# ExaScience/bpmf

Hardware: AMD Instinct MI355X
Metric: user+item column samples/sec per Gibbs iter; test RMSE vs reference (higher is better)
Workload: dtype f64

## Files before the change

### bpmf_amd/csrc/args.h

```cpp
#pragma once
#include <hip/hip_runtime.h>
#include <stdint.h>

#include "blob.h"

namespace bpmf {

__host__ __device__ constexpr int tri_off(int i) { return 2 * ((i >> 1) + 1) * ((i >> 1) + (i & 1)); }

template <int K>
struct Geo {
    static constexpr int NT = (K + 15) / 16;
    static constexpr int NTRI = NT * (NT + 1) / 2;
    static constexpr int PART = NTRI * 256 + NT * 16;
    static constexpr int WPS = K <= 32 ? 4 : 2;
    static constexpr int C = 64 / K;
    static constexpr int NP = K / 2;
    static constexpr int PLEN = tri_off(K);
    static constexpr int SLOT = PLEN + 2 * K;
    static constexpr int LDS_WORDS = C * SLOT + 2 * C;
};

template <int K>
struct Geo44 {
    static constexpr int NG = K / 4;
    static constexpr int NB = NG * (NG + 1) / 2;
    static constexpr int NL = K / 8;
    static constexpr int PART = (NB + NG) * 64;
    __host__ __device__ static constexpr int idx(int g, int x) { return 8 * (g >> 1) + 2 * x + (g & 1); }
};

struct SampleArgs {
    const int32_t *rowidx;
    const double *vals;
    const int32_t *wi_col;
    const int64_t *wi_p0;
    const int32_t *wi_len;
    const int32_t *wi_mc;
    const int32_t *wi_chunk;
    const int32_t *mc_slot0;
    const int32_t *mc_nchunks;
    unsigned *mc_count;
    double *partials;
    int nwork;
    const double *other_items;
    const double *zero_row;
    double *items;
    int64_t col_from;
    const double *LambdaF;
    const double *Lmu;
    const double *mu;
    const float *lf32;
    const double *prop_lambda;
    uint32_t diag_only;
    unsigned long long *fail;
    double mean_rating;
    double alpha;
    uint32_t iter_plus_1;
    int ktrue;
    const unsigned *gate_flag;
    unsigned gate_want;
    unsigned long long *tmo;
    unsigned long long wait_ticks;
    unsigned long long *stamps;
    uint32_t ablate;
};

struct FusedArgs {
    const unsigned *gate_host; unsigned gate_want; const double *src_host; double *dst; int n; unsigned *dflag; unsigned dval;
    int nstat; const double *st_items; int64_t st_c0, st_c1; double *st_partials; const unsigned long long *st_fail;
    double *st_out; unsigned *st_ticket; unsigned *st_flag; unsigned st_seq;
    unsigned long long *st_tmo;
// ... 51 lines not shown
```

### bpmf_amd/csrc/capi_side.hip

```cpp
#include "capi_internal.h"

namespace bpmf_capi {

int build_schedule(bpmf_hip_side *s, const int64_t *colptr)
{
    const int64_t nloc = s->to - s->from;
    const int K = s->ctx->K;
    const int mode_env = env_int("BPMF_HIP_MODE", -1);
    const bool f32 = s->ctx->dtype == BPMF_HIP_F32;
    const bool big = K == 128;
    if (big) s->mode = 5;
    else if (K == 64) s->mode = 4;
    else s->mode = (mode_env == 1 || mode_env == 3) ? mode_env : (nloc >= 20000 ? 3 : 1);
    int chunk = env_int("BPMF_HIP_CHUNK", 0);
    if (chunk <= 0) {
        const int64_t simds = (int64_t)s->ctx->num_cu * 4;
        int64_t c = s->mode == 4 ? (s->nnz * 9) / (simds * 16) : (s->mode == 5 ? (s->nnz * (f32 ? 3 : 6)) / (simds * 7) : s->nnz / simds);
        c = (c + 63) / 64 * 64;
        const int64_t lo = s->mode == 4 ? 256 : (s->mode == 5 ? 256 : 16 * K);
        chunk = (int)std::min<int64_t>(std::max<int64_t>(c, lo), 65536);
        if (s->mode == 3) chunk = std::max(chunk / 4, 4 * K);
    }
    chunk = (chunk + 15) / 16 * 16;
    s->chunk = chunk;

    struct Item { int32_t col; int64_t p0; int32_t len; int32_t mc; int32_t chunk; int64_t cost; };
    std::vector<Item> items;
    items.reserve((size_t)nloc + (size_t)(s->nnz / chunk) + 16);
    std::vector<int32_t> mc_slot0, mc_nch;
    const int64_t fin_cost = 32;
    int32_t slots = 0;
    for (int64_t c = 0; c < nloc; ++c) {
        const int64_t p0 = colptr[c], n = colptr[c + 1] - colptr[c];
        if (n < 0) return fail(BPMF_HIP_EINVAL, "colptr is not monotone");
        if (n <= chunk) {
// ... 60 lines not shown
        if (pfmax > 0) {
            size_t at[18] = {0};
            for (const Item &it : items)
                if (it.mc < 0 && it.len <= pfmax) at[it.len + 1]++;
            for (int n = 1; n <= pfmax + 1; ++n) at[n] += at[n - 1];
            lc.resize(at[pfmax + 1]); ll.resize(at[pfmax + 1]); lp.resize(at[pfmax + 1]);
            if (pfmax >= 3) s->pf_class[1] = (int)at[4];
            if (pfmax >= 6) s->pf_class[2] = (int)at[7];
            for (const Item &it : items)
                if (it.mc < 0 && it.len <= pfmax) { const size_t q = at[it.len]++; lc[q] = it.col; ll[q] = it.len; lp[q] = it.p0; }
        }
        s->pf_ratings = s->pf_ratings2 = 0;
        for (int32_t l : ll) { s->pf_ratings += l; s->pf_ratings2 += (int64_t)l * l; }
        if (pfmax < 3) s->pf_class[1] = (int)lc.size();
        if (pfmax < 6) s->pf_class[2] = (int)lc.size();
        s->pf_class[3] = (int)lc.size();
        for (const Item &it : items)
            if (!(it.mc < 0 && it.len <= nlr)) { hc.push_back(it.col); hl.push_back(it.len); hm.push_back(it.mc); hk.push_back(it.chunk); hp.push_back(it.p0); }
        if (nlr > 0 && (int64_t)lc.size() * 2 >= nloc && !lc.empty()) {
            s->lr_n = (int)lc.size(); s->hv_nwork = (int)hc.size();
            if (s->pf_class[3] > 0 && (rc = dev_upload<double>(&s->d_pf_q, nullptr, (size_t)s->nrows * K))) return rc;
            if ((rc = dev_upload(&s->d_lr_col, lc.data(), lc.size())) || (rc = dev_upload(&s->d_lr_len, ll.data(), ll.size())) ||
                (rc = dev_upload(&s->d_lr_p0, lp.data(), lp.size())) || (rc = dev_upload(&s->d_hv_col, hc.data(), hc.size())) ||
                (rc = dev_upload(&s->d_hv_len, hl.data(), hl.size())) || (rc = dev_upload(&s->d_hv_mc, hm.data(), hm.size())) ||
                (rc = dev_upload(&s->d_hv_chunk, hk.data(), hk.size())) || (rc = dev_upload(&s->d_hv_p0, hp.data(), hp.size())))
                return rc;
        }
    }
    if ((rc = dev_upload(&s->d_wi_col, wcol.data(), nw))) return rc;
    if ((rc = dev_upload(&s->d_wi_len, wlen.data(), nw))) return rc;
    if ((rc = dev_upload(&s->d_wi_mc, wmc.data(), nw))) return rc;
    if ((rc = dev_upload(&s->d_wi_chunk, wchunk.data(), nw))) return rc;
    if ((rc = dev_upload(&s->d_wi_p0, wp0.data(), nw))) return rc;
    if ((rc = dev_upload(&s->d_mc_slot0, mc_slot0.data(), mc_slot0.size()))) return rc;
    if ((rc = dev_upload(&s->d_mc_nch, mc_nch.data(), mc_nch.size()))) return rc;
    {
        std::vector<unsigned> zeros(std::max<size_t>(mc_slot0.size(), 8 * 32), 0u);
        if ((rc = dev_upload(&s->d_mc_count, zeros.data(), std::max<size_t>(mc_slot0.size(), 1)))) return rc;
    }
    if (big) {
        s->nstat_waves = (int)std::max<int64_t>(1, std::min<int64_t>((nloc + 63) / 64, 32));
        if ((rc = dev_upload<double>(&s->d_stat_partials, nullptr, (size_t)s->nstat_waves * blob::stat_partial_words(K)))) return rc;
        if ((rc = dev_upload<double>(&s->d_partials, nullptr, (size_t)slots * part_words_rt(K, f32)))) return rc;
        return 0;
    }
    const size_t pw = part_words_rt(K, false);
    if ((rc = dev_upload<double>(&s->d_partials, nullptr, (size_t)slots * pw))) return rc;
    s->nstat_waves = (int)std::max<int64_t>(1, std::min<int64_t>((nloc + 31) / 32, (int64_t)s->ctx->num_cu * (nloc > 100000 ? 8 : 2)));
    if (nloc < 20000) s->nstat_waves = (int)std::max<int64_t>(1, std::min<int64_t>(s->nstat_waves, std::max<int64_t>((nloc + 159) / 160, 24)));
    s->nstat_wg = (nloc > 100000) ? (int)std::min<int64_t>((nloc + 127) / 128, (int64_t)s->ctx->num_cu * 2) : 0;
    if ((rc = dev_upload<double>(&s->d_stat_partials, nullptr, (size_t)std::max(s->nstat_waves, 2 * s->nstat_wg) * pw))) return rc;
    return 0;
}

void free_schedule(bpmf_hip_side *s)
{
    void **ptrs[] = {(void **)&s->d_wi_col, (void **)&s->d_wi_len, (void **)&s->d_wi_mc, (void **)&s->d_wi_chunk, (void **)&s->d_wi_p0,
                     (void **)&s->d_mc_slot0, (void **)&s->d_mc_nch, (void **)&s->d_mc_count, (void **)&s->d_partials, (void **)&s->d_stat_partials,
                     (void **)&s->d_lr_col, (void **)&s->d_lr_len, (void **)&s->d_lr_p0, (void **)&s->d_hv_col, (void **)&s->d_hv_len,
                     (void **)&s->d_hv_mc, (void **)&s->d_hv_chunk, (void **)&s->d_hv_p0, (void **)&s->d_pf_q};
    for (void **p : ptrs) if (*p) { (void)hipFree(*p); *p = nullptr; }
    s->lr_n = s->hv_nwork = 0;
}


static int side_create_common(bpmf_hip_ctx *ctx, int64_t ncols, int64_t nrows, int64_t from, int64_t to,
                              const int64_t *colptr, const int32_t *rowidx, const double *vals, bool dev_arrays,
                              double mean_rating, bpmf_hip_side **out)
{
    if (!out) return fail(BPMF_HIP_EINVAL, "side_create: out is NULL");
    *out = nullptr;
    if (!ctx || !colptr || ncols <= 0 || nrows <= 0 || from < 0 || to < from || to > ncols)
        return fail(BPMF_HIP_EINVAL, "side_create: bad argument");
    const int64_t nloc = to - from;
    if (nloc >= (int64_t)1 << 31) return fail(BPMF_HIP_EINVAL, "side_create: more than 2^31-1 local columns");
    if (colptr[0] != 0) return fail(BPMF_HIP_EINVAL, "side_create: colptr[0] must be 0 (pass the local slice)");
    const int64_t nnz = colptr[nloc];
    if (nnz > 0 && (!rowidx || !vals)) return fail(BPMF_HIP_EINVAL, "side_create: NULL rowidx/vals");
    HIP_TRY(hipSetDevice(ctx->device));
    if (!dev_arrays) {
        for (int64_t p = 0; p < nnz; ++p)
            if (rowidx[p] < 0 || rowidx[p] >= nrows) return fail(BPMF_HIP_EINVAL, "side_create: row index out of range");
    }
    bpmf_hip_side *s = new (std::nothrow) bpmf_hip_side();
    if (!s) return fail(BPMF_HIP_ENOMEM, "side_create: out of host memory");
    s->ctx = ctx; s->ncols = ncols; s->nrows = nrows; s->from = from; s->to = to; s->nnz = nnz; s->mean_rating = mean_rating;
    int rc = 0;
    if (dev_arrays) {
        s->d_rowidx = const_cast<int32_t *>(rowidx); s->d_vals = const_cast<double *>(vals); s->own_csc = false;
    } else {
        if ((rc = dev_upload(&s->d_rowidx, rowidx, (size_t)nnz)) || (rc = dev_upload(&s->d_vals, vals, (size_t)nnz))) { bpmf_hip_side_destroy(s); return rc; }
    }
    const size_t words = (size_t)ctx->K * (size_t)ncols;
    const size_t esz = ctx->dtype == BPMF_HIP_F32 ? sizeof(float) : sizeof(double);
    hipError_t e = hipMalloc((void **)&s->d_items, words * esz);
// ... 41 lines not shown
        fprintf(stderr, "[bpmf_hip] side %04x: previous sampler's end -> this sampler's start: %.2f us (mean of %lld timed launches)\n",
                (unsigned)((uintptr_t)s >> 4) & 0xFFFF, s->tot_gap_ms / (double)s->n_gap * 1e3, (long long)s->n_gap);
    {
        std::lock_guard<std::mutex> lk(s->ctx->launch_mutex);
        for (bpmf_hip_side *sd : s->ctx->sides)
            if (sd->deferred_eval && sd->deferred_eval->side == s) {
                sd->deferred_eval->deferred = false; sd->deferred_eval->cancelled = true;
                sd->deferred_eval = nullptr;
            }
    }
    flush_deferred(s->deferred_eval);
    (void)bounded_stream_sync(s->ctx, s->ctx->stream, __func__);
    if (s->saux) {
        (void)bounded_stream_sync(s->ctx, s->saux, __func__); (void)hipStreamDestroy(s->saux);
        std::lock_guard<std::mutex> lk(s->ctx->launch_mutex);
        auto &v = s->ctx->sides;
        v.erase(std::remove(v.begin(), v.end(), s), v.end());
    }
    if (s->sx) { (void)bounded_stream_sync(s->ctx, s->sx, __func__); (void)hipStreamDestroy(s->sx); }
    for (hipEvent_t e : s->sub_ev) if (e) (void)hipEventDestroy(e);
    if (s->sx_done) (void)hipEventDestroy(s->sx_done);
    if (s->ev_stat_go) (void)hipEventDestroy(s->ev_stat_go);
    if (s->own_csc) { if (s->d_rowidx) (void)hipFree(s->d_rowidx); if (s->d_vals) (void)hipFree(s->d_vals); }
    if (s->own_items && s->d_items) (void)hipFree(s->d_items);
    if (s->d_items_alt) (void)hipFree(s->d_items_alt);
    if (s->d_prop) (void)hipFree(s->d_prop);
    s->probit.reset(); s->censor.reset(); s->link.reset(); s->ring.reset(); s->sse.reset(); s->d_colptr.reset();
    if (s->d_aggr_mu) (void)hipFree(s->d_aggr_mu);
    if (s->d_aggr_lambda) (void)hipFree(s->d_aggr_lambda);
    void *ptrs[] = {s->d_wi_col, s->d_wi_len, s->d_wi_mc, s->d_wi_chunk, s->d_wi_p0, s->d_mc_slot0, s->d_mc_nch, s->d_mc_count, s->d_partials,
                    s->d_stat_partials, s->a_d_in,
                    s->d_lr_col, s->d_lr_len, s->d_lr_p0, s->d_hv_col, s->d_hv_len, s->d_hv_mc, s->d_hv_chunk, s->d_hv_p0,
                    s->d_conn_send, s->d_conn_recv, s->d_conn_sbuf, s->d_conn_rbuf, s->d_pf_q,
                    s->d_prec, s->d_t_colptr, s->d_t_rowidx, s->d_t_vals, s->d_t_order};
    for (void *p : ptrs) if (p) (void)hipFree(p);
    if (s->a_h_in) (void)hipHostFree(s->a_h_in);
    if (s->a_h_out) (void)hipHostFree(s->a_h_out);
    for (auto &set : s->evs) for (hipEvent_t e : set) if (e) (void)hipEventDestroy(e);
    if (s->a_gate) (void)hipHostFree(s->a_gate);
    if (s->a_ticket) (void)hipFree(s->a_ticket);
    if (s->a_dflag) (void)hipFree(s->a_dflag);
    if (s->a_d_red) (void)hipFree(s->a_d_red);
    delete s;
    return BPMF_HIP_OK;
}

int require_single_gpu(const char *who, const bpmf_hip_ctx *c, const bpmf_hip_side *a, const bpmf_hip_side *b, const char *tail)
{
    if (!c->comm && !sharded(a) && !(b && sharded(b))) return 0;
    return fail(BPMF_HIP_EINVAL, std::string(who) + (b ? ": needs both sides whole on one GPU" : ": needs the side whole on one GPU") + tail);
}

int ensure_colptr(bpmf_hip_side *s) { return s->d_colptr ? 0 : s->d_colptr.upload(s->h_colptr.data(), s->h_colptr.size()); }

extern "C" int64_t bpmf_hip_live_device_bytes(void) { return g_live_bytes.load(std::memory_order_relaxed); }

void pad_square(int Kt, int K, const double *src, double *dst, double diag)
{
    for (int j = 0; j < K; ++j)
        for (int i = 0; i < K; ++i)
            dst[(size_t)j * K + i] = (i < Kt && j < Kt) ? src[(size_t)j * Kt + i] : ((i == j) ? diag : 0.0);
}
void unpad_square(int Kt, int K, const double *src, double *dst)
{
    for (int j = 0; j < Kt; ++j) memcpy(dst + (size_t)j * Kt, src + (size_t)j * K, sizeof(double) * Kt);
}

// ... 107 lines not shown
        std::vector<float> tmp(words, 0.0f);
        for (size_t c = 0; c < n; ++c)
            for (size_t i = 0; i < Kt; ++i) tmp[c * K + i] = (float)h[c * Kt + i];
        HIP_TRY(hipMemcpy(s->d_items, tmp.data(), words * sizeof(float), hipMemcpyHostToDevice));
        return BPMF_HIP_OK;
    }
    if (Kt == K) HIP_TRY(hipMemcpy(s->d_items, h, words * sizeof(double), hipMemcpyHostToDevice));
    else {
        HIP_TRY(hipMemset(s->d_items, 0, words * sizeof(double)));
        HIP_TRY(hipMemcpy2D(s->d_items, K * sizeof(double), h, Kt * sizeof(double), Kt * sizeof(double), n, hipMemcpyHostToDevice));
    }
    return BPMF_HIP_OK;
}

extern "C" int bpmf_hip_side_kernel_name(const bpmf_hip_side *s, char *buf, int n)
{
    if (!s || !buf || n <= 0) return fail(BPMF_HIP_EINVAL, "side_kernel_name: bad argument");
    const bpmf_hip_ctx *c = s->ctx;
    const int K = c->K;
    const std::string k = std::to_string(K);
    const bool dist = c->comm != nullptr && !s->bounds.empty();
    const bool fusable = !dist && !s->reduce_on && env_int("BPMF_HIP_FUSED", 1) != 0 && s->nwork > 0;
    std::string name;
    if (s->reduce_on) name = "k_sample_prec<" + k + "> + k_precompute<" + k + ">";
    else if (c->dtype == BPMF_HIP_F32) name = "k_sample_wg2<128,2>";
    else if (K == 128) name = "k_sample_wg2<128,4,double>";
    else if (K == 64) {
        if (s->lr_n > 0 && !s->d_prop && !c->diag_only) {
            static const char *nb[3] = {"3", "6", "16"};
            for (int pc = 0; pc < 3; ++pc)
                if (s->pf_class[pc + 1] > s->pf_class[pc]) name += std::string(name.empty() ? "" : " + ") + "k_sample_pf<64," + nb[pc] + ">";
            if (s->hv_nwork > 0) name += " + k_sample_slab<64>";
        } else name = (fusable && s->lr_n == 0 && s->nsub <= 1) ? "k_sample1s<64>" : "k_sample_slab<64>";
    } else name = (s->mode == 3 ? "k_sample4<" : "k_sample1<") + k + ">";
    snprintf(buf, (size_t)n, "%s", name.c_str());
    return BPMF_HIP_OK;
}

extern "C" int bpmf_hip_side_kernel_resources(bpmf_hip_side *s, int64_t *out, int max_kernels, char *names, int names_len)
{
    if (!s || !out || max_kernels <= 0) return fail(BPMF_HIP_EINVAL, "side_kernel_resources: bad argument");
    bpmf_hip_ctx *c = s->ctx;
    HIP_TRY(hipSetDevice(c->device));
    if (s->reduce_on) return 0;
    bpmf_launch::Probe pr;
    bpmf_launch::probe() = &pr;
    const int rc = BPMF_DISPATCH_K(c->K, (bpmf_launch::sampler_into<KK, FF>(s, s->d_items, s, 0, 1.0, c->d_in, c->stream, nullptr, nullptr)));
    bpmf_launch::probe() = nullptr;
    if (rc) return rc;
    std::string all;
    const int n = std::min(pr.n, max_kernels);
    for (int i = 0; i < n; ++i) {
        for (int j = 0; j < 4; ++j) out[4 * i + j] = pr.v[i][j];
        std::string nm = pr.name[i];
        for (const char *strip : {"bpmf::", "(", ")"}) { size_t p; while ((p = nm.find(strip)) != std::string::npos) nm.erase(p, strlen(strip)); }
        all += (i ? ";" : "") + nm;
    }
    if (names && names_len > 0) snprintf(names, (size_t)names_len, "%s", all.c_str());
    return n;
}

extern "C" int bpmf_hip_side_schedule_info(const bpmf_hip_side *s, int64_t *out, int n)
{
    if (!s || !out || n < 16) return fail(BPMF_HIP_EINVAL, "side_schedule_info: bad argument (16 words)");
    for (int i = 0; i < n; ++i) out[i] = 0;
    out[0] = s->mode; out[1] = s->nwork; out[2] = s->nslots; out[3] = s->nmulti;
    out[4] = s->lr_n; out[5] = s->lr_n > 0 ? s->hv_nwork : s->nwork;
// ... 33 lines not shown
```

### bpmf_amd/csrc/kernels.h

```cpp
#pragma once
#include <hip/hip_runtime.h>
#include <stdint.h>

#include "philox.h"
#include "args.h"

namespace bpmf {

typedef double d4 __attribute__((ext_vector_type(4)));

__device__ __forceinline__ d4 mfma16(double a, double b, d4 c)
{
    return __builtin_amdgcn_mfma_f64_16x16x4f64(a, b, c, 0, 0, 0);
}

__device__ __forceinline__ double mfma44(double a, double b, double c)
{
    return __builtin_amdgcn_mfma_f64_4x4x4f64(a, b, c, 0, 0, 0);
}

template <int K>
struct Rot44 {
    static constexpr int NT = K / 16;
    __host__ __device__ static constexpr int nrot(int TI, int TJ) { return TI == TJ ? 3 : 4; }
// ... 362 lines not shown
        for (int g = 0; g < NG; ++g)
#pragma unroll
            for (int g2 = g; g2 < NG; ++g2, ++blk) acc[blk] = mfma44(R[g], R[g2], acc[blk]);
    };
    if (len <= 0) return;
    dd2 yA[NL], yB[NL];
    double wA, wB = 0.0;
    gather(cur, 0, yA, wA);
    int b0 = 0;
    for (; b0 + 64 < len; b0 += 64) {
        const IdxBlock nn = load_idx_block(rowidx, vals, b0 + 128, lane, len, zero_row);
        gather(cur, 1, yB, wB);
        contract(yA, wA);
        gather(cur, 2, yA, wA);
        contract(yB, wB);
        gather(cur, 3, yB, wB);
        contract(yA, wA);
        gather(nxt, 0, yA, wA);
        contract(yB, wB);
        cur = nxt;
        nxt = nn;
    }
    const int ng = (len - b0 + 15) >> 4;
    if (ng > 1) gather(cur, 1, yB, wB);
    contract(yA, wA);
    if (ng > 1) {
        if (ng > 2) gather(cur, 2, yA, wA);
        contract(yB, wB);
        if (ng > 2) {
            if (ng > 3) gather(cur, 3, yB, wB);
            contract(yA, wA);
            if (ng > 3) contract(yB, wB);
        }
    }
}

template <int K>
__device__ __forceinline__ void assemble44(double (&acc)[Geo44<K>::NB], double (&rr)[Geo44<K>::NG], double *sA, double *sb,
                                           int LD, int lane)
{
    using G = Geo44<K>;
    constexpr int NG = G::NG;
    static_assert(NG % 2 == 0, "block rows are written in pairs");
    const int i = lane >> 4, b = (lane >> 2) & 3, j = lane & 3;
    auto blk = [](int g, int g2) constexpr { return g * NG - (g * (g - 1)) / 2 + (g2 - g); };
    double *up = sA + (2 * i) * LD + 2 * j;
    double *lo = sA + (2 * j) * LD + 2 * i;
#pragma unroll
    for (int g = 0; g < NG; g += 2) {
#pragma unroll
        for (int t = blk(g, g); t < blk(g + 1, NG - 1) + 1; ++t) {
            const double v = row_ror_add<0x128>(acc[t]);
            acc[t] = row_ror_add<0x124>(v);
        }
        if (b == 0) {
            up[G::idx(g + 1, 0) * LD + G::idx(g + 1, 0)] = acc[blk(g + 1, g + 1)];
#pragma unroll
            for (int g2 = g; g2 < NG; g2 += 2) {
                double2 v; v.x = acc[blk(g, g2)]; v.y = acc[blk(g, g2 + 1)];
                *reinterpret_cast<double2 *>(&up[G::idx(g, 0) * LD + G::idx(g2, 0)]) = v;
                if (g2 > g) {
                    double2 w; w.x = acc[blk(g + 1, g2)]; w.y = acc[blk(g + 1, g2 + 1)];
                    *reinterpret_cast<double2 *>(&up[G::idx(g + 1, 0) * LD + G::idx(g2, 0)]) = w;
                }
            }
        } else if (b == 1) {
// ... 298 lines not shown

    double bi = yi + zi;
    const double my_dinv = 1.0 / sA[roff(i) + i];
    constexpr int BB = K < 8 ? K : 8;
#pragma unroll
    for (int kb = K - BB; kb >= 0; kb -= BB) {
        double lv[BB];
#pragma unroll
        for (int t = 0; t < BB; ++t) lv[t] = *((i < kb + t) ? &sA[roff(kb + t) + i] : szero);
#pragma unroll
        for (int t = BB - 1; t >= 0; --t) {
            const int k = kb + t;
            if (k == 0) continue;
            const double xk = bcast(bi * my_dinv, k);
            bi = fma(-lv[t], xk, bi);
        }
    }
    const double xi = bi * my_dinv;

    if (lane < K) a.items[(size_t)idx * K + lane] = xi;
    const bool bad = !(fabs(xi) <= 1.79769313486231570815e+308);
    if (__any(bad) && lane == 0) atomicMin(a.fail, (unsigned long long)idx);
}

template <int K>
__device__ __forceinline__ void colstats_body(int w, const double *__restrict__ items, int64_t c0, int64_t c1, int nwaves,
                                              double *partials, const unsigned long long *__restrict__ fail_in,
                                              double *__restrict__ out, unsigned *ticket, unsigned *flag, unsigned seq,
                                              unsigned long long *tmo, unsigned long long wait_ticks, double *img);
__device__ __forceinline__ void gate_stage_body(int block, int nblocks, const unsigned *gate_host, unsigned want, const double *src_host,
                                                double *__restrict__ dst, int n, unsigned *dflag, unsigned dval,
                                                unsigned long long *tmo, unsigned long long wait_ticks);

template <int K>
__global__ __launch_bounds__(64, Geo1<K>::WPS) void k_sample1(SampleArgs a, FusedArgs f)
{
    __shared__ __attribute__((aligned(16))) double lds[Geo1<K>::LDS_WORDS];
    const int lane = threadIdx.x;
    int bid = blockIdx.x;
    if (f.gate_host) {
        if (bid == 0) { gate_stage_body(0, 1, f.gate_host, f.gate_want, f.src_host, f.dst, f.n, f.dflag, f.dval, a.tmo, a.wait_ticks); return; }
        --bid;
    }
    if (bid < f.nstat) {
        colstats_body<K>(bid, f.st_items, f.st_c0, f.st_c1, f.nstat, f.st_partials, f.st_fail, f.st_out, f.st_ticket, f.st_flag, f.st_seq,
                         f.st_tmo, a.wait_ticks, lds);
        return;
    }
    const int w = bid - f.nstat;
    const int col = a.wi_col[w];
    const int64_t p0 = a.wi_p0[w];
    const int len = a.wi_len[w];
    const int mc = a.wi_mc[w];

    const int glen = (ablate_bits(a) & 2u) ? 0 : len;
    const IdxBlock ib0 = load_idx_block(a.rowidx + p0, a.vals + p0, 0, lane, glen, a.zero_row);
    const IdxBlock ib1 = load_idx_block(a.rowidx + p0, a.vals + p0, 64, lane, glen, a.zero_row);

    if (mc < 0 && !(ablate_bits(a) & 1u))
        draw_normals<K>(sample_counter(a.col_from + col, a.ktrue, a.iter_plus_1), a.ktrue, lds + Geo1<K>::AWORDS + K, lane, K);

    static_assert(K <= 32, "k_sample1: K <= 32 (K = 64 runs the slab form, K = 128 the workgroup form)");
    {
        using G4 = Geo44<K>;
        constexpr int NB = G4::NB, NG = G4::NG, PART = G4::PART;
        double acc[NB], rr[NG];
#pragma unroll
        for (int t = 0; t < NB; ++t) acc[t] = 0.0;
#pragma unroll
        for (int t = 0; t < NG; ++t) rr[t] = 0.0;
        gram_chunk44<K>(a.rowidx + p0, a.vals + p0, glen, a.other_items, a.zero_row, a.mean_rating, a.alpha, ib0, ib1, acc, rr, lane,
                        (ablate_bits(a) & 4u) ? 63 : -1);
        if (ablate_bits(a) & 1u) {
            double v = rr[0];
#pragma unroll
            for (int t = 0; t < NB; ++t) v += acc[t];
            if (mc < 0 && lane < K) a.items[(size_t)(a.col_from + col) * K + lane] = v;
            return;
        }
        if (mc >= 0) {
            const int nch = a.mc_nchunks[mc];
            double *pbase = a.partials + (size_t)a.mc_slot0[mc] * PART;
            double *p = pbase + (size_t)a.wi_chunk[w] * PART;
#pragma unroll
            for (int t = 0; t < NB; ++t) __hip_atomic_store(&p[t * 64 + lane], acc[t], BPMF_RLX_AGENT);
#pragma unroll
            for (int t = 0; t < NG; ++t) __hip_atomic_store(&p[(NB + t) * 64 + lane], rr[t], BPMF_RLX_AGENT);
            asm volatile("s_waitcnt vmcnt(0)" ::: "memory");
            unsigned t = 0;
            if (lane == 0) t = __hip_atomic_fetch_add(&a.mc_count[mc], 1u, BPMF_RLX_AGENT);
            t = __builtin_amdgcn_readfirstlane(t);
            if ((int)t != nch - 1) return;
            if (lane == 0) __hip_atomic_store(&a.mc_count[mc], 0u, BPMF_RLX_AGENT);
#pragma unroll
            for (int t2 = 0; t2 < NB; ++t2) acc[t2] = 0.0;
#pragma unroll
            for (int t2 = 0; t2 < NG; ++t2) rr[t2] = 0.0;
            for (int ch = 0; ch < nch; ++ch) {
                const double *pc = pbase + (size_t)ch * PART;
                double tmp[NB + NG];
#pragma unroll
                for (int t2 = 0; t2 < NB + NG; ++t2) tmp[t2] = __hip_atomic_load(&pc[t2 * 64 + lane], BPMF_RLX_AGENT);
#pragma unroll
                for (int t2 = 0; t2 < NB; ++t2) acc[t2] += tmp[t2];
#pragma unroll
                for (int t2 = 0; t2 < NG; ++t2) rr[t2] += tmp[NB + t2];
            }
        }
        wait_params(a);
        finish_single<K>(a, col, lds, lane, mc < 0,
                         [&](double *sA, double *sb, int LD, int ln) { assemble44<K>(acc, rr, sA, sb, LD, ln); });
    }
}

#define BPMF_RLX_SYSTEM __ATOMIC_RELAXED, __HIP_MEMORY_SCOPE_SYSTEM
__device__ __forceinline__ void publish_when_last(unsigned *ticket, unsigned nblocks, unsigned *flag_host, unsigned seq,
                                                  unsigned *rearm = nullptr, unsigned *rearm2 = nullptr)
{
    asm volatile("s_waitcnt vmcnt(0)" ::: "memory");
    __syncthreads();
    if (threadIdx.x == 0) {
        const unsigned t = __hip_atomic_fetch_add(ticket, 1u, BPMF_RLX_AGENT);
        if (t == nblocks - 1) {
            __hip_atomic_store(ticket, 0u, BPMF_RLX_AGENT);
            if (rearm) __hip_atomic_store(rearm, 0u, BPMF_RLX_AGENT);
            if (rearm2) __hip_atomic_store(rearm2, 0u, BPMF_RLX_AGENT);
            __hip_atomic_store(flag_host, seq, BPMF_RLX_SYSTEM);
        }
    }
}

template <int K>
constexpr bool kColstatsRot = (K == 64);

template <int K>
__device__ __forceinline__ void colstats_accumulate(const double *__restrict__ items, int64_t b, int64_t e,
                                                    d4 (&acc)[Geo<K>::NTRI], double (&r)[Geo<K>::NT], int lane, double *img,
                                                    const int32_t *__restrict__ list = nullptr, int64_t c0 = 0)
{
    constexpr int NT = Geo<K>::NT;
    constexpr bool ROT = kColstatsRot<K>;
    const int kq = lane >> 4, li = lane & 15;
    double C[ROT ? Rot44<K>::NACC : 1];
#pragma unroll
    for (int t = 0; t < (ROT ? Rot44<K>::NACC : 1); ++t) C[t] = 0.0;
// ... 478 lines not shown
```

### bpmf_amd/csrc/launch_impl.h

```cpp
#pragma once
#include "launch.h"
#include "kernels.h"
#include "kernels_f32.h"
#include "kernels_q4.h"
#include "kernels_slab.h"

namespace bpmf_launch {


template <int K, bool F32>
int sampler_into(bpmf_hip_side *self, double *out_items, const bpmf_hip_side *other, int iter, double alpha, double *d_in, hipStream_t st,
                        hipEvent_t ev_start, hipEvent_t ev_stop)
{
    using namespace bpmf;
    bpmf_hip_ctx *c = self->ctx;
    SampleArgs a = blob_args(self, out_items, d_in, iter, alpha);
    const double *vals = self->probit ? self->probit->z.get() : self->censor ? self->censor->z.get() : self->link ? self->link->r.get() : self->d_vals;
    a.rowidx = self->d_rowidx; a.vals = vals;
    const int w0 = self->item_n >= 0 ? self->item_off : 0, nwork = self->item_n >= 0 ? self->item_n : self->nwork;
    a.wi_col = self->d_wi_col + w0; a.wi_p0 = self->d_wi_p0 + w0; a.wi_len = self->d_wi_len + w0; a.wi_mc = self->d_wi_mc + w0; a.wi_chunk = self->d_wi_chunk + w0;
    a.mc_slot0 = self->d_mc_slot0; a.mc_nchunks = self->d_mc_nch; a.mc_count = self->d_mc_count;
    a.partials = self->d_partials; a.nwork = nwork;
    a.other_items = other->d_items;
    a.ablate = c->ablate; a.stamps = c->d_stamps;
// ... 33 lines not shown
            if (self->pf_class[3] > self->pf_class[0] && self->d_pf_q) {
                const int grid = (int)std::max<int64_t>(1, std::min<int64_t>((self->nrows + 7) / 8, (int64_t)c->num_cu * 4));
                k64_pf_prepare(grid, st, started ? nullptr : ev_start, l.S0t, other->d_items, self->nrows, self->d_pf_q);
                started = true;
            }
            int last_pf = -1;
            for (int pc = 0; pc < 3; ++pc) if (self->pf_class[pc + 1] > self->pf_class[pc]) last_pf = pc;
            for (int pc = 0; pc < 3; ++pc) {
                const int n0 = self->pf_class[pc], n1 = self->pf_class[pc + 1];
                if (n1 <= n0) continue;
                LrArgs lc = l;
                lc.col = l.col + n0; lc.p0 = l.p0 + n0; lc.len = l.len + n0; lc.nitems = n1 - n0;
                hipEvent_t e0 = started ? nullptr : ev_start, e1 = pc == last_pf ? ev_stop : nullptr;
                started = true;
                const int grid = std::max(1, std::min((n1 - n0 + 31) / 32, c->num_cu * 4));
                k64_pf(pc, grid, st, e0, e1, lc);
            }
            return 0;
        }
        if (nwork > 0) {
            const FusedArgs &f = self->cur_fused;
            if (f.gate_host || f.nstat) {
                const dim3 grid((unsigned)(nwork + (f.gate_host ? 1 : 0) + f.nstat));
                BPMF_LAUNCH(k_sample1s<K>, grid, dim3(64), st, ev_start, ev_stop, a, f);
            } else {
                k64_slab(nwork, st, ev_start, ev_stop, a);
            }
        }
        return 0;
    } else {
    if (nwork > 0) {
        const FusedArgs &f = self->cur_fused;
        const dim3 grid((unsigned)(nwork + (f.gate_host ? 1 : 0) + f.nstat));
        BPMF_LAUNCH(k_sample1<K>, grid, dim3(64), st, ev_start, ev_stop, a, f);
    }
    return 0;
    }
    }
}

template <int K, bool F32>
int exchange(bpmf_hip_side *self, hipStream_t st, int sub)
{
    bpmf_hip_ctx *c = self->ctx;
    if (!(c->comm != nullptr && !self->bounds.empty())) return 0;
    COMM_ALIVE_OR_FAIL(c, "exchange");
    const bool f32 = c->dtype == BPMF_HIP_F32;
    const ncclDataType_t ty = f32 ? ncclFloat : ncclDouble;
    const size_t esz = f32 ? sizeof(float) : sizeof(double);
    char *items = reinterpret_cast<char *>(self->d_items);
    Rccl *R = rccl();
    if (!self->conn_send_ptr.empty()) {
        if constexpr (F32) return fail(BPMF_HIP_EINVAL, "the connectivity-aware exchange is fp64 only");
        else {
        if (sub >= 0 && self->nsub > 1 && sub != self->nsub - 1) return 0;
        const int64_t ns = self->conn_send_ptr.back(), nr = self->conn_recv_ptr.back();
        constexpr int P = K / 2;
        if (ns > 0)
            hipLaunchKernelGGL(bpmf::k_pack_cols<K>, dim3((unsigned)((ns * P + 255) / 256)), dim3(256), 0, st,
                               (const double *)self->d_items, (const int32_t *)self->d_conn_send, ns, self->d_conn_sbuf);
        NcclGroup group(R);
        NCCL_TRY(group.start());
        for (int r = 0; r < c->nranks; ++r) {
            const int64_t s0 = self->conn_send_ptr[(size_t)r], s1 = self->conn_send_ptr[(size_t)r + 1];
            const int64_t r0 = self->conn_recv_ptr[(size_t)r], r1 = self->conn_recv_ptr[(size_t)r + 1];
            if (s1 > s0) NCCL_TRY(R->Send(self->d_conn_sbuf + (size_t)s0 * K, (size_t)(s1 - s0) * K, ncclDouble, r, c->comm, st));
            if (r1 > r0) NCCL_TRY(R->Recv(self->d_conn_rbuf + (size_t)r0 * K, (size_t)(r1 - r0) * K, ncclDouble, r, c->comm, st));
// ... 133 lines not shown
```

### bpmf_amd/csrc/state.h

```cpp
#pragma once
#include <hip/hip_runtime.h>
#include <hip/hip_ext.h>
#include <rccl/rccl.h>

#include <algorithm>
#include <atomic>
#include <chrono>
#include <condition_variable>
#include <mutex>
#include <thread>
#include <cstdio>
#include <cstdlib>
#include <cstring>
#include <cmath>
#include <deque>
#include <limits>
#include <new>
#include <numeric>
#include <string>
#include <vector>

#include "../../include/bpmf_hip.h"
#include "args.h"

// ... 132 lines not shown
    double *d_zero = nullptr;
    hipEvent_t ev[3] = {nullptr, nullptr, nullptr};
};

struct bpmf_hip_side {
    bpmf_hip_ctx *ctx = nullptr;
    int64_t ncols = 0, nrows = 0, from = 0, to = 0, nnz = 0;
    double mean_rating = 0.0;
    int32_t *d_rowidx = nullptr; double *d_vals = nullptr; bool own_csc = true;
    double *d_items = nullptr; bool own_items = true;
    double *d_items_alt = nullptr; bool items_exposed = false; int cur_buf = 0;
    struct Reader { struct bpmf_hip_test *t = nullptr; unsigned seq = 0; } readers[2];
    struct bpmf_hip_test *deferred_eval = nullptr;
    double *d_aggr_mu = nullptr, *d_aggr_lambda = nullptr;
    double *d_prop = nullptr;
    std::unique_ptr<bpmf_probit> probit;
    std::unique_ptr<bpmf_censor> censor;
    std::unique_ptr<bpmf_link> link;
    std::unique_ptr<bpmf_ring> ring;
    std::unique_ptr<bpmf_sse> sse;
    DevBuf<int64_t> d_colptr;
    bool probit_latent_queued = false;
    int nwork = 0, nmulti = 0, nslots = 0, mode = 0;
    int chunk = 0;
    int lr_n = 0, hv_nwork = 0;
    int64_t pf_ratings2 = 0;
    int64_t pf_ratings = 0;
    int pf_class[4] = {0, 0, 0, 0};
    double *d_pf_q = nullptr;
    int32_t *d_lr_col = nullptr, *d_lr_len = nullptr; int64_t *d_lr_p0 = nullptr;
    int32_t *d_hv_col = nullptr, *d_hv_len = nullptr, *d_hv_mc = nullptr, *d_hv_chunk = nullptr; int64_t *d_hv_p0 = nullptr;
    int32_t *d_wi_col = nullptr, *d_wi_len = nullptr, *d_wi_mc = nullptr, *d_wi_chunk = nullptr;
    int64_t *d_wi_p0 = nullptr;
    int32_t *d_mc_slot0 = nullptr, *d_mc_nch = nullptr;
    unsigned *d_mc_count = nullptr;
    double *d_partials = nullptr;
    int nstat_waves = 0;
    int nstat_wg = 0;
    hipEvent_t ev_stat_go = nullptr;
    double *d_stat_partials = nullptr;
    std::vector<int64_t> bounds;
    int nsub = 1;
    int stale_k = 0;
    bool stale_explicit = false;
    bool stale_primed = false;
    std::vector<int64_t> sub_bounds;
    std::vector<int> sub_item_off;
    int item_off = 0, item_n = -1;
    hipStream_t sx = nullptr;
    hipEvent_t sub_ev[8] = {nullptr, nullptr, nullptr, nullptr, nullptr, nullptr, nullptr, nullptr}, sx_done = nullptr;
    bool reduce_on = false;
    double *d_prec = nullptr;
    int64_t *d_t_colptr = nullptr; int32_t *d_t_rowidx = nullptr; double *d_t_vals = nullptr; int32_t *d_t_order = nullptr;
    std::vector<int64_t> h_colptr;
    std::vector<int64_t> conn_send_ptr, conn_recv_ptr;
    int32_t *d_conn_send = nullptr, *d_conn_recv = nullptr;
    double *d_conn_sbuf = nullptr, *d_conn_rbuf = nullptr;
    int64_t failed_column = -1;
    bool pending = false;
    float last_sample_ms = 0.f, last_reduce_ms = 0.f;
    bool timing_valid = true;
    double *a_h_in = nullptr, *a_h_in_dev = nullptr, *a_d_in = nullptr;
    double *a_h_out = nullptr, *a_h_out_dev = nullptr;
    bpmf::FusedArgs cur_fused{};
    bpmf::StatRiders cur_riders{};
    std::atomic<hipEvent_t> stats_ev[2] = {{nullptr}, {nullptr}};
// ... 11 lines not shown
    std::thread worker;
    std::mutex wm;
    std::condition_variable wcv;
    std::deque<Job> jobs;
    int in_flight = 0;
    bool wstop = false;
    int async_rc = 0;
    std::string async_msg;
    int gate_iter = -2;
    double tot_sample_ms = 0.0, tot_reduce_ms = 0.0;
    long long n_launches = 0;
    int iter = -1;
    double norm = 0.0;
    int collected_iter = -1;
    double norm_hist[8] = {0, 0, 0, 0, 0, 0, 0, 0};
    std::vector<double> cov, hp_mu, hp_LambdaU, hp_LambdaF;
    std::vector<double> nx_mu, nx_LambdaU, nx_LambdaF;
    int nx_iter = -2;
    std::vector<double> rd_au, rd_z;
    int rd_iter = -2;
    struct Predraw {
        static constexpr int DEPTH = 8;
        struct Slot { std::vector<double> au, z; int iter = -1; };
        Slot slot[DEPTH];
        std::vector<std::thread> threads;
        std::mutex m;
        std::condition_variable cv;
        int next = 0;
        int consumed = -1;
        bool stop = false;
    } predraw;
};

struct bpmf_hip_test {
    bpmf_hip_side *side = nullptr;
    int64_t nnz = 0;
    int32_t *d_tcol = nullptr, *d_trow = nullptr;
    double *d_tval = nullptr, *d_pavg = nullptr, *d_pm2 = nullptr, *d_partial = nullptr;
    int64_t nblocks = 0;
    int wg = 256;
    int64_t global_nnz = -1;
    double *h_res = nullptr, *h_res_dev = nullptr;
    unsigned *d_ticket = nullptr;
    unsigned seq = 0, done_seq = 0;
    bool launched = false;
    hipEvent_t ev_in = nullptr, ev_done[2] = {nullptr, nullptr}, in_ev = nullptr;
    hipStream_t pstream = nullptr;
    bool deferred = false, cancelled = false; int def_n = 0; struct bpmf_hip_side *def_other = nullptr;
    const void *def_self_items = nullptr, *def_other_items = nullptr;
    struct bpmf_hip_test *twin = nullptr, *owner = nullptr;
    int32_t *d_twin_perm = nullptr;
    std::vector<int32_t> h_col, h_row;
    double *d_prob_sum = nullptr; int prob_n = 0;
};

inline int check_timeout(double *h_blob, int K, std::string *msg)
{
    unsigned long long *w = blob::tmo_word(h_blob, K);
    const unsigned long long v = __atomic_load_n(w, __ATOMIC_ACQUIRE);
    if (!v) return 0;
    __atomic_store_n(w, 0ull, __ATOMIC_RELEASE);
    *msg = std::string("device wait timed out: ") + kTimeoutWhat[v < 5 ? v : 0];
    return BPMF_HIP_ENODEV;
}

inline int check_probit(bpmf_hip_side *s, std::string *msg)
// ... 52 lines not shown
```

Measured before the change: 101.0 million.

## Precompute packed gather-record stream for mode-1 f64 sampling kernel

At setup, builds an interleaved per-work-item array of 16-byte records (pre-scaled row offset plus mean-centred rating), padded to groups of 16, for the small-K f64 mode-1 path. A new templated kernel variant reads one vector load per record instead of separate rowidx and vals loads with index multiply and mean subtraction, pipelining two groups ahead. This is meant to cut index/value load latency and instruction count in the Gram accumulation loop. It costs extra device memory for a duplicate copy of the ratings and depends on vals being the original device values.

Result: faster. 105.4 million, median of 6 (+4.4%).

```diff
diff --git a/bpmf_amd/csrc/args.h b/bpmf_amd/csrc/args.h
--- a/bpmf_amd/csrc/args.h
+++ b/bpmf_amd/csrc/args.h
@@ -30,6 +30,14 @@
     __host__ __device__ static constexpr int idx(int g, int x) { return 8 * (g >> 1) + 2 * x + (g & 1); }
 };
 
+struct GatherRec {
+    int32_t off;
+    int32_t unused;
+    double d;
+};
+static_assert(sizeof(GatherRec) == 16, "one 16-byte load per record");
+constexpr int kGatherTailGroups = 4;
+
 struct SampleArgs {
     const int32_t *rowidx;
     const double *vals;
@@ -38,6 +46,9 @@
     const int32_t *wi_len;
     const int32_t *wi_mc;
     const int32_t *wi_chunk;
+    const GatherRec *gs_rec;
+    const int32_t *gs_g0;
+    const int32_t *gs_ng;
     const int32_t *mc_slot0;
     const int32_t *mc_nchunks;
     unsigned *mc_count;
diff --git a/bpmf_amd/csrc/capi_side.hip b/bpmf_amd/csrc/capi_side.hip
--- a/bpmf_amd/csrc/capi_side.hip
+++ b/bpmf_amd/csrc/capi_side.hip
@@ -1,6 +1,45 @@
 #include "capi_internal.h"
 
 namespace bpmf_capi {
+
+static int build_gather_stream(bpmf_hip_side *s, const std::vector<int64_t> &wp0, const std::vector<int32_t> &wlen)
+{
+    const int K = s->ctx->K;
+    if (s->mode != 1 || K > 32 || s->ctx->dtype != BPMF_HIP_F64 || env_int("BPMF_HIP_GATHER_STREAM", 1) == 0) return 0;
+    if (s->nrows * (int64_t)(K / 2) > (int64_t)INT32_MAX) return 0;
+    const size_t nw = wlen.size();
+    int64_t groups = 0;
+    for (size_t i = 0; i < nw; ++i) groups += (wlen[i] + 15) / 16;
+    groups += bpmf::kGatherTailGroups;
+    if (groups > (int64_t)INT32_MAX / 16) return 0;
+    std::vector<int32_t> ri((size_t)s->nnz);
+    std::vector<double> rv((size_t)s->nnz);
+    if (s->nnz > 0) {
+        HIP_TRY(hipMemcpy(ri.data(), s->d_rowidx, (size_t)s->nnz * sizeof(int32_t), hipMemcpyDeviceToHost));
+        HIP_TRY(hipMemcpy(rv.data(), s->d_vals, (size_t)s->nnz * sizeof(double), hipMemcpyDeviceToHost));
+    }
+    const bpmf::GatherRec pad = {-1, 0, 0.0};
+    std::vector<bpmf::GatherRec> rec((size_t)groups * 16, pad);
+    std::vector<int32_t> g0(nw), ng(nw);
+    int64_t g = 0;
+    for (size_t i = 0; i < nw; ++i) {
+        g0[i] = (int32_t)g; ng[i] = (wlen[i] + 15) / 16;
+        bpmf::GatherRec *out = rec.data() + (size_t)g * 16;
+        for (int32_t q = 0; q < wlen[i]; ++q) {
+            const int64_t p = wp0[i] + q;
+            if (ri[(size_t)p] < 0 || ri[(size_t)p] >= s->nrows) return fail(BPMF_HIP_EINVAL, "side_create: row index out of range");
+            out[q].off = (int32_t)((int64_t)ri[(size_t)p] * (K / 2));
+            out[q].d = rv[(size_t)p] - s->mean_rating;
+        }
+        g += ng[i];
+    }
+    int rc;
+    if ((rc = dev_upload(&s->d_gs_rec, rec.data(), rec.size()))) return rc;
+    if ((rc = dev_upload(&s->d_gs_g0, g0.data(), nw))) return rc;
+    if ((rc = dev_upload(&s->d_gs_ng, ng.data(), nw))) return rc;
+    s->gs_groups = groups;
+    return 0;
+}
 
 int build_schedule(bpmf_hip_side *s, const int64_t *colptr)
 {
@@ -127,6 +166,7 @@
     if ((rc = dev_upload(&s->d_wi_mc, wmc.data(), nw))) return rc;
     if ((rc = dev_upload(&s->d_wi_chunk, wchunk.data(), nw))) return rc;
     if ((rc = dev_upload(&s->d_wi_p0, wp0.data(), nw))) return rc;
+    if ((rc = build_gather_stream(s, wp0, wlen))) return rc;
     if ((rc = dev_upload(&s->d_mc_slot0, mc_slot0.data(), mc_slot0.size()))) return rc;
     if ((rc = dev_upload(&s->d_mc_nch, mc_nch.data(), mc_nch.size()))) return rc;
     {
@@ -153,9 +193,10 @@
     void **ptrs[] = {(void **)&s->d_wi_col, (void **)&s->d_wi_len, (void **)&s->d_wi_mc, (void **)&s->d_wi_chunk, (void **)&s->d_wi_p0,
                      (void **)&s->d_mc_slot0, (void **)&s->d_mc_nch, (void **)&s->d_mc_count, (void **)&s->d_partials, (void **)&s->d_stat_partials,
                      (void **)&s->d_lr_col, (void **)&s->d_lr_len, (void **)&s->d_lr_p0, (void **)&s->d_hv_col, (void **)&s->d_hv_len,
-                     (void **)&s->d_hv_mc, (void **)&s->d_hv_chunk, (void **)&s->d_hv_p0, (void **)&s->d_pf_q};
+                     (void **)&s->d_hv_mc, (void **)&s->d_hv_chunk, (void **)&s->d_hv_p0, (void **)&s->d_pf_q,
+                     (void **)&s->d_gs_rec, (void **)&s->d_gs_g0, (void **)&s->d_gs_ng};
     for (void **p : ptrs) if (*p) { (void)hipFree(*p); *p = nullptr; }
-    s->lr_n = s->hv_nwork = 0;
+    s->lr_n = s->hv_nwork = 0; s->gs_groups = 0;
 }
 
 
@@ -263,7 +304,7 @@
                     s->d_stat_partials, s->a_d_in,
                     s->d_lr_col, s->d_lr_len, s->d_lr_p0, s->d_hv_col, s->d_hv_len, s->d_hv_mc, s->d_hv_chunk, s->d_hv_p0,
                     s->d_conn_send, s->d_conn_recv, s->d_conn_sbuf, s->d_conn_rbuf, s->d_pf_q,
-                    s->d_prec, s->d_t_colptr, s->d_t_rowidx, s->d_t_vals, s->d_t_order};
+                    s->d_prec, s->d_t_colptr, s->d_t_rowidx, s->d_t_vals, s->d_t_order, s->d_gs_rec, s->d_gs_g0, s->d_gs_ng};
     for (void *p : ptrs) if (p) (void)hipFree(p);
     if (s->a_h_in) (void)hipHostFree(s->a_h_in);
     if (s->a_h_out) (void)hipHostFree(s->a_h_out);
@@ -437,7 +478,7 @@
                 if (s->pf_class[pc + 1] > s->pf_class[pc]) name += std::string(name.empty() ? "" : " + ") + "k_sample_pf<64," + nb[pc] + ">";
             if (s->hv_nwork > 0) name += " + k_sample_slab<64>";
         } else name = (fusable && s->lr_n == 0 && s->nsub <= 1) ? "k_sample1s<64>" : "k_sample_slab<64>";
-    } else name = (s->mode == 3 ? "k_sample4<" : "k_sample1<") + k + ">";
+    } else name = (s->mode == 3 ? "k_sample4<" : uses_gather_stream(s) ? "k_sample1<" : "k_sample1i<") + k + ">";
     snprintf(buf, (size_t)n, "%s", name.c_str());
     return BPMF_HIP_OK;
 }
diff --git a/bpmf_amd/csrc/kernels.h b/bpmf_amd/csrc/kernels.h
--- a/bpmf_amd/csrc/kernels.h
+++ b/bpmf_amd/csrc/kernels.h
@@ -418,6 +418,65 @@
             contract(yA, wA);
             if (ng > 3) contract(yB, wB);
         }
+    }
+}
+
+typedef double gs_raw __attribute__((ext_vector_type(2)));
+__device__ __forceinline__ gs_raw load_gs_rec(const GatherRec *__restrict__ rec, int g, unsigned slot_bytes)
+{
+    return *reinterpret_cast<const gs_raw *>(reinterpret_cast<const char *>(rec + 16 * g) + slot_bytes);
+}
+
+template <int K>
+__device__ __forceinline__ void gram_stream44(const GatherRec *__restrict__ rec, int ng, const double *__restrict__ other,
+                                              const double *__restrict__ zero_row, double alpha, gs_raw r0, gs_raw r1, unsigned slot_bytes,
+                                              double (&acc)[Geo44<K>::NB], double (&rr)[Geo44<K>::NG], int lane)
+{
+    using G = Geo44<K>;
+    constexpr int NG = G::NG, NL = G::NL;
+    typedef double dd2 __attribute__((ext_vector_type(2)));
+    const int x = lane & 3;
+    const dd2 *ox = reinterpret_cast<const dd2 *>(other + 2 * x), *zx = reinterpret_cast<const dd2 *>(zero_row + 2 * x);
+    auto gather = [&](const gs_raw &rc, dd2 (&yy)[NL], double &ww) {
+        const int off = (int)__builtin_bit_cast(long long, rc.x);
+        ww = rc.y * alpha;
+        const dd2 *p = (off >= 0) ? ox + off : zx;
+#pragma unroll
+        for (int h = 0; h < NL; ++h) yy[h] = p[4 * h];
+    };
+    auto contract = [&](const dd2 (&yy)[NL], double ww) {
+        double R[NG];
+#pragma unroll
+        for (int h = 0; h < NL; ++h) { R[2 * h] = yy[h].x; R[2 * h + 1] = yy[h].y; }
+#pragma unroll
+        for (int g = 0; g < NG; ++g) rr[g] = fma(R[g], ww, rr[g]);
+        int blk = 0;
+#pragma unroll
+        for (int g = 0; g < NG; ++g)
+#pragma unroll
+            for (int g2 = g; g2 < NG; ++g2, ++blk) acc[blk] = mfma44(R[g], R[g2], acc[blk]);
+    };
+    if (ng <= 0) return;
+    dd2 yA[NL], yB[NL];
+    double wA, wB = 0.0;
+    gather(r0, yA, wA);
+    r0 = load_gs_rec(rec, 2, slot_bytes);
+    if (ng > 1) gather(r1, yB, wB);
+    r1 = load_gs_rec(rec, 3, slot_bytes);
+    contract(yA, wA);
+    int g = 1;
+    for (; g + 2 < ng; g += 2) {
+        gather(r0, yA, wA);
+        r0 = load_gs_rec(rec, g + 3, slot_bytes);
+        contract(yB, wB);
+        gather(r1, yB, wB);
+        r1 = load_gs_rec(rec, g + 4, slot_bytes);
+        contract(yA, wA);
+    }
+    if (g < ng) {
+        if (g + 1 < ng) gather(r0, yA, wA);
+        contract(yB, wB);
+        if (g + 1 < ng) contract(yA, wA);
     }
 }
 
@@ -782,10 +841,9 @@
                                                 double *__restrict__ dst, int n, unsigned *dflag, unsigned dval,
                                                 unsigned long long *tmo, unsigned long long wait_ticks);
 
-template <int K>
-__global__ __launch_bounds__(64, Geo1<K>::WPS) void k_sample1(SampleArgs a, FusedArgs f)
-{
-    __shared__ __attribute__((aligned(16))) double lds[Geo1<K>::LDS_WORDS];
+template <int K, bool GS>
+__device__ __forceinline__ void sample1_body(const SampleArgs &a, const FusedArgs &f, double *lds)
+{
     const int lane = threadIdx.x;
     int bid = blockIdx.x;
     if (f.gate_host) {
@@ -804,8 +862,20 @@
     const int mc = a.wi_mc[w];
 
     const int glen = (ablate_bits(a) & 2u) ? 0 : len;
-    const IdxBlock ib0 = load_idx_block(a.rowidx + p0, a.vals + p0, 0, lane, glen, a.zero_row);
-    const IdxBlock ib1 = load_idx_block(a.rowidx + p0, a.vals + p0, 64, lane, glen, a.zero_row);
+    IdxBlock ib0{}, ib1{};
+    gs_raw gr0{}, gr1{};
+    const GatherRec *rec = nullptr;
+    const unsigned slot_bytes = 16u * ((unsigned)lane >> 2);
+    int ng = 0;
+    if constexpr (GS) {
+        rec = a.gs_rec + (size_t)a.gs_g0[w] * 16;
+        ng = (ablate_bits(a) & 2u) ? 0 : a.gs_ng[w];
+        gr0 = load_gs_rec(rec, 0, slot_bytes);
+        gr1 = load_gs_rec(rec, 1, slot_bytes);
+    } else {
+        ib0 = load_idx_block(a.rowidx + p0, a.vals + p0, 0, lane, glen, a.zero_row);
+        ib1 = load_idx_block(a.rowidx + p0, a.vals + p0, 64, lane, glen, a.zero_row);
+    }
 
     if (mc < 0 && !(ablate_bits(a) & 1u))
         draw_normals<K>(sample_counter(a.col_from + col, a.ktrue, a.iter_plus_1), a.ktrue, lds + Geo1<K>::AWORDS + K, lane, K);
@@ -819,8 +889,11 @@
         for (int t = 0; t < NB; ++t) acc[t] = 0.0;
 #pragma unroll
         for (int t = 0; t < NG; ++t) rr[t] = 0.0;
-        gram_chunk44<K>(a.rowidx + p0, a.vals + p0, glen, a.other_items, a.zero_row, a.mean_rating, a.alpha, ib0, ib1, acc, rr, lane,
-                        (ablate_bits(a) & 4u) ? 63 : -1);
+        if constexpr (GS)
+            gram_stream44<K>(rec, ng, a.other_items, a.zero_row, a.alpha, gr0, gr1, slot_bytes, acc, rr, lane);
+        else
+            gram_chunk44<K>(a.rowidx + p0, a.vals + p0, glen, a.other_items, a.zero_row, a.mean_rating, a.alpha, ib0, ib1, acc, rr, lane,
+                            (ablate_bits(a) & 4u) ? 63 : -1);
         if (ablate_bits(a) & 1u) {
             double v = rr[0];
 #pragma unroll
@@ -861,6 +934,20 @@
         finish_single<K>(a, col, lds, lane, mc < 0,
                          [&](double *sA, double *sb, int LD, int ln) { assemble44<K>(acc, rr, sA, sb, LD, ln); });
     }
+}
+
+template <int K>
+__global__ __launch_bounds__(64, Geo1<K>::WPS) void k_sample1(SampleArgs a, FusedArgs f)
+{
+    __shared__ __attribute__((aligned(16))) double lds[Geo1<K>::LDS_WORDS];
+    sample1_body<K, true>(a, f, lds);
+}
+
+template <int K>
+__global__ __launch_bounds__(64, Geo1<K>::WPS) void k_sample1i(SampleArgs a, FusedArgs f)
+{
+    __shared__ __attribute__((aligned(16))) double lds[Geo1<K>::LDS_WORDS];
+    sample1_body<K, false>(a, f, lds);
 }
 
 #define BPMF_RLX_SYSTEM __ATOMIC_RELAXED, __HIP_MEMORY_SCOPE_SYSTEM
diff --git a/bpmf_amd/csrc/launch_impl.h b/bpmf_amd/csrc/launch_impl.h
--- a/bpmf_amd/csrc/launch_impl.h
+++ b/bpmf_amd/csrc/launch_impl.h
@@ -89,7 +89,12 @@
     if (nwork > 0) {
         const FusedArgs &f = self->cur_fused;
         const dim3 grid((unsigned)(nwork + (f.gate_host ? 1 : 0) + f.nstat));
-        BPMF_LAUNCH(k_sample1<K>, grid, dim3(64), st, ev_start, ev_stop, a, f);
+        if (uses_gather_stream(self) && vals == self->d_vals) {
+            a.gs_rec = self->d_gs_rec; a.gs_g0 = self->d_gs_g0 + w0; a.gs_ng = self->d_gs_ng + w0;
+            BPMF_LAUNCH(k_sample1<K>, grid, dim3(64), st, ev_start, ev_stop, a, f);
+        } else {
+            BPMF_LAUNCH(k_sample1i<K>, grid, dim3(64), st, ev_start, ev_stop, a, f);
+        }
     }
     return 0;
     }
diff --git a/bpmf_amd/csrc/state.h b/bpmf_amd/csrc/state.h
--- a/bpmf_amd/csrc/state.h
+++ b/bpmf_amd/csrc/state.h
@@ -188,6 +188,9 @@
     int32_t *d_hv_col = nullptr, *d_hv_len = nullptr, *d_hv_mc = nullptr, *d_hv_chunk = nullptr; int64_t *d_hv_p0 = nullptr;
     int32_t *d_wi_col = nullptr, *d_wi_len = nullptr, *d_wi_mc = nullptr, *d_wi_chunk = nullptr;
     int64_t *d_wi_p0 = nullptr;
+    bpmf::GatherRec *d_gs_rec = nullptr;
+    int32_t *d_gs_g0 = nullptr, *d_gs_ng = nullptr;
+    int64_t gs_groups = 0;
     int32_t *d_mc_slot0 = nullptr, *d_mc_nch = nullptr;
     unsigned *d_mc_count = nullptr;
     double *d_partials = nullptr;
@@ -265,6 +268,11 @@
     } predraw;
 };
 
+inline bool uses_gather_stream(const bpmf_hip_side *s)
+{
+    return s->d_gs_rec && s->mode == 1 && !s->probit && !s->censor && !s->link && !(s->ctx->ablate & 4u);
+}
+
 struct bpmf_hip_test {
     bpmf_hip_side *side = nullptr;
     int64_t nnz = 0;
```
